# the-lay/voltools

Hardware: AMD Instinct MI355X
Metric: Mvoxels/s, 512^3 f32 filt_bspline StaticVolume transform (resident source, device output) (higher is better)
Workload: dtype f32; 1 GPU; 512^3 float32 filt_bspline, StaticVolume resident in HBM, rotate((0,i,0)) rzxz sweep, output= device buffer; lds_bytes=34816, kernel=8, resident_bytes=1660944384, angles=i

## Files before the change

include/voltools_hip.h:

```cpp
#ifndef VOLTOOLS_HIP_H
#define VOLTOOLS_HIP_H

#include <stddef.h>
#include <stdint.h>

#ifdef __cplusplus
extern "C" {
#endif

enum vt_interp {
    VT_LINEAR = 0,
    VT_BSPLINE = 1,
    VT_BSPLINE_SIMPLE = 2,
    VT_FILT_BSPLINE = 3,
    VT_FILT_BSPLINE_SIMPLE = 4
};

enum vt_flags {
    VT_OUT_DEVICE = 1,
    VT_KEEP_OUTSIDE = 2,
    VT_FORCE_DIRECT = 4,
    VT_FORCE_TILED = 8,
    VT_NO_ZSEP = 16,
    VT_NO_MARCH = 32,
    VT_NO_ZPAIR = 64,
    VT_NO_PACKED = 128,
    VT_FORCE_PACKED = 256,
    VT_FORCE_XSWAP = 512,
    VT_NO_RSWAP = 1024,
    VT_ONESHOT_EDGE_SCIPY = 4096,
    VT_NO_QUAD = 2048,
    VT_NO_BLOCK = 8192,
    VT_NO_ZFIR = 16384,
    VT_NO_REORIENT = 32768,
    VT_NO_ROWS = 65536,
    VT_NO_PLANSHARE = 131072,
    VT_ACCUMULATE = 262144,
    VT_PLACE_DENSE = 524288
};

enum vt_create_flags {
    VT_SRC_DEVICE = 1,
    VT_SLAB_LO_INTERIOR = 2,
    VT_SLAB_HI_INTERIOR = 4,
    VT_EDGE_SCIPY = 16,
    VT_SRC_DEFERRED = 8,
    VT_STACK = 32
};

enum vt_error {
    VT_OK = 0,
    VT_EINVAL = 10001,
    VT_ENODEV = 10002,
    VT_ENOMEM = 10003,
    VT_EUNSUPPORTED = 10004
};

typedef struct vt_volume vt_volume_t;

typedef struct vt_volume_info {
    int32_t device;
    int32_t interp;
    int32_t depth, height, width;
    int32_t out_depth, out_height, out_width;
    int32_t last_kernel;
    int32_t last_tile[3];
    int32_t last_lds_dims[3];
    int32_t last_lds_bytes;
    int32_t last_grid;
    float   prefilter_ms;
    uint64_t resident_bytes;
    float   copies_ms;
    int32_t copies_built;
    int32_t copies_evicted;
    uint64_t max_resident_bytes;
} vt_volume_info_t;

int vt_device_count(int* count);
int vt_device_name(int dev, char* buf, int buflen);
int vt_device_props(int dev, int* cu_count, int* lds_bytes_per_block, uint64_t* hbm_bytes);
int vt_device_synchronize(int dev);

int vt_malloc(int dev, size_t bytes, void** dptr);
int vt_free(int dev, void* dptr);
int vt_memset_zero(int dev, void* dptr, size_t bytes);
int vt_memcpy_h2d(int dev, void* dptr, const void* hptr, size_t bytes);
int vt_memcpy_d2h(int dev, void* hptr, const void* dptr, size_t bytes);
int vt_memcpy_d2d(int dev, void* dst, const void* src, size_t bytes);
int vt_host_register(int dev, void* ptr, size_t bytes);
int vt_host_unregister(int dev, void* ptr);
int vt_device_trim(int dev);

int vt_volume_create(int dev, int depth, int height, int width, int interp,
                     const float* data, int create_flags, vt_volume_t** out);

int vt_volume_create_slab(int dev, int local_depth, int height, int width, int interp,
                          const float* data, int create_flags,
                          int64_t plane0, int64_t global_depth, int64_t out_plane0, int out_depth,
                          vt_volume_t** out);

int vt_volume_upload_planes(vt_volume_t* vol, int first_plane, int nplanes, const float* data, int flags);
int vt_volume_finalize(vt_volume_t* vol);

int vt_has_legacy_kernels(void);

int vt_volume_release_copies(vt_volume_t* vol, uint64_t* freed_bytes);
int vt_volume_set_max_resident(vt_volume_t* vol, uint64_t bytes);
int vt_volume_destroy(vt_volume_t* vol);
int vt_volume_info(const vt_volume_t* vol, vt_volume_info_t* info);
int vt_volume_stream(const vt_volume_t* vol, void** hip_stream);
int vt_volume_sync(vt_volume_t* vol);

int vt_volume_set_output_shape(vt_volume_t* vol, int out_depth, int out_height, int out_width);

int vt_volume_affine(vt_volume_t* vol, const float* m4x4, float* out, int flags);
int vt_volume_affine_f64(vt_volume_t* vol, const double* m4x4, float* out, int flags);

int vt_volume_affine_batch(vt_volume_t* vol, int n, const float* m4x4s, float* out, int flags);

int vt_volume_extract(vt_volume_t* vol, int n, const float* m4x4s,
                      int box_d, int box_h, int box_w, float* out, int flags);
// ... 73 lines not shown
```

voltools_amd/_native.py:

```python
import ctypes
import os
from typing import Optional, Tuple

import numpy as np

_HERE = os.path.dirname(os.path.abspath(__file__))
LIB_PATH = os.environ.get('VT_LIB') or os.path.join(_HERE, 'lib', 'libvoltools_hip.so')

INTERP_CODES = {'linear': 0, 'bspline': 1, 'bspline_simple': 2, 'filt_bspline': 3, 'filt_bspline_simple': 4}

OUT_DEVICE, KEEP_OUTSIDE, FORCE_DIRECT, FORCE_TILED, NO_ZSEP, NO_MARCH, NO_ZPAIR, NO_PACKED, FORCE_PACKED, FORCE_XSWAP, NO_RSWAP, NO_QUAD, ONESHOT_EDGE_SCIPY, NO_BLOCK, NO_ZFIR, NO_REORIENT, NO_ROWS, NO_PLANSHARE, ACCUMULATE, PLACE_DENSE = 1, 2, 4, 8, 16, 32, 64, 128, 256, 512, 1024, 2048, 4096, 8192, 16384, 32768, 65536, 131072, 262144, 524288
SRC_DEVICE, SLAB_LO_INTERIOR, SLAB_HI_INTERIOR, SRC_DEFERRED, EDGE_SCIPY, STACK = 1, 2, 4, 8, 16, 32

SYMBOLS = [
    'vt_device_count', 'vt_device_name', 'vt_device_props', 'vt_device_synchronize',
    'vt_malloc', 'vt_free', 'vt_memset_zero', 'vt_memcpy_h2d', 'vt_memcpy_d2h', 'vt_memcpy_d2d',
    'vt_host_register', 'vt_host_unregister', 'vt_device_trim',
    'vt_volume_create', 'vt_volume_create_slab', 'vt_volume_upload_planes', 'vt_volume_finalize', 'vt_volume_destroy', 'vt_volume_info', 'vt_volume_stream',
    'vt_volume_sync', 'vt_volume_set_output_shape', 'vt_volume_affine', 'vt_volume_affine_f64',
    'vt_volume_project', 'vt_volume_project_f64', 'vt_volume_affine_batch',
    'vt_timer_start', 'vt_timer_stop', 'vt_prefilter_inplace', 'vt_affine_oneshot',
    'vt_last_error', 'vt_version', 'vt_has_legacy_kernels', 'vt_volume_release_copies', 'vt_volume_set_max_resident',
    'vt_volume_extract', 'vt_volume_extract_f64', 'vt_volume_project_batch', 'vt_volume_project_batch_f64',
    'vt_volume_extract_sum', 'vt_volume_extract_sum_f64', 'vt_volume_extract_dot', 'vt_volume_extract_dot_f64',
    'vt_volume_extract_dot_multi', 'vt_volume_extract_dot_multi_f64',
    'vt_volume_extract_sum_multi', 'vt_volume_extract_sum_multi_f64',
    'vt_volume_place', 'vt_volume_place_f64', 'vt_volume_backproject', 'vt_volume_backproject_f64',
    'vt_volume_backproject_boxes', 'vt_volume_backproject_boxes_f64',
    'vt_volume_warp', 'vt_volume_warp_f64',
]


class VolumeInfo(ctypes.Structure):
    _fields_ = [('device', ctypes.c_int32), ('interp', ctypes.c_int32),
                ('depth', ctypes.c_int32), ('height', ctypes.c_int32), ('width', ctypes.c_int32),
                ('out_depth', ctypes.c_int32), ('out_height', ctypes.c_int32), ('out_width', ctypes.c_int32),
                ('last_kernel', ctypes.c_int32), ('last_tile', ctypes.c_int32 * 3),
                ('last_lds_dims', ctypes.c_int32 * 3), ('last_lds_bytes', ctypes.c_int32),
                ('last_grid', ctypes.c_int32), ('prefilter_ms', ctypes.c_float),
                ('resident_bytes', ctypes.c_uint64), ('copies_ms', ctypes.c_float), ('copies_built', ctypes.c_int32),
                ('copies_evicted', ctypes.c_int32), ('max_resident_bytes', ctypes.c_uint64)]


_lib = None


def _preload_hip_runtime():
    import importlib.util
    import sys
    if os.environ.get('VT_HIP_RUNTIME', '') == 'system' or 'torch' in sys.modules:
        return
    try:
        spec = importlib.util.find_spec('torch')
    except (ImportError, ValueError):
        spec = None
    if spec is None or not spec.submodule_search_locations:
        return
    cand = os.path.join(list(spec.submodule_search_locations)[0], 'lib', 'libamdhip64.so')
    if os.path.exists(cand):
        try:
            ctypes.CDLL(cand, mode=ctypes.RTLD_GLOBAL)
        except OSError:
            pass


def load():
    global _lib
    if _lib is not None:
        return _lib
    if not os.path.exists(LIB_PATH):
        raise OSError(f'{LIB_PATH} not found (run __graft_entry__.build())')
    _preload_hip_runtime()
    L = ctypes.CDLL(LIB_PATH)
    c_int, c_void_p, c_size_t, c_i64 = ctypes.c_int, ctypes.c_void_p, ctypes.c_size_t, ctypes.c_int64
    P = ctypes.POINTER
    L.vt_has_legacy_kernels.argtypes = []
    L.vt_device_count.argtypes = [P(c_int)]
    L.vt_device_name.argtypes = [c_int, ctypes.c_char_p, c_int]
    L.vt_device_props.argtypes = [c_int, P(c_int), P(c_int), P(ctypes.c_uint64)]
    L.vt_device_synchronize.argtypes = [c_int]
    L.vt_malloc.argtypes = [c_int, c_size_t, P(c_void_p)]
    L.vt_free.argtypes = [c_int, c_void_p]
    L.vt_memset_zero.argtypes = [c_int, c_void_p, c_size_t]
    L.vt_memcpy_h2d.argtypes = [c_int, c_void_p, c_void_p, c_size_t]
    L.vt_memcpy_d2h.argtypes = [c_int, c_void_p, c_void_p, c_size_t]
    L.vt_host_register.argtypes = [c_int, c_void_p, c_size_t]
    L.vt_host_unregister.argtypes = [c_int, c_void_p]
    L.vt_device_trim.argtypes = [c_int]
    L.vt_memcpy_d2d.argtypes = [c_int, c_void_p, c_void_p, c_size_t]
    L.vt_volume_create.argtypes = [c_int, c_int, c_int, c_int, c_int, c_void_p, c_int, P(c_void_p)]
    L.vt_volume_create_slab.argtypes = [c_int, c_int, c_int, c_int, c_int, c_void_p, c_int,
                                        c_i64, c_i64, c_i64, c_int, P(c_void_p)]
    L.vt_volume_upload_planes.argtypes = [c_void_p, c_int, c_int, c_void_p, c_int]
    L.vt_volume_finalize.argtypes = [c_void_p]
# ... 262 lines not shown
```

voltools_amd/csrc/vt_kernels_block.hip:

```cpp
#include "vt_internal.h"
#include "vt_device.h"

#include <algorithm>
#include <type_traits>

namespace vt {

typedef float v2f __attribute__((ext_vector_type(2)));

constexpr int kBlkTD = 8, kBlkTW = 16;
constexpr int block_max_it(int th) { return th == 16 ? 20 : 13; }

template <int OFF>
__device__ __forceinline__ void lds_read_b64(v2f& r, unsigned a)
{
    asm volatile("ds_read_b64 %0, %1 offset:%2" : "=v"(r) : "v"(a), "n"(OFF));
}

__device__ __forceinline__ v2f pk_fma(v2f a, float w, v2f c) { return __builtin_elementwise_fma(a, (v2f)(w), c); }

__device__ __forceinline__ void bspline_weights_pk(float f, v2f& w30, v2f& w12)
{
    const v2f fg = {f, 1.0f - f};
    const v2f sq = fg * fg;
// ... 14 lines not shown
    } else {
        v2f a30, a12;
        bspline_weights_pk(fx, a30, a12); wx[0] = a30.y; wx[1] = a12.x; wx[2] = a12.y; wx[3] = a30.x;
        bspline_weights_pk(fy, a30, a12); wy[0] = a30.y; wy[1] = a12.x; wy[2] = a12.y; wy[3] = a30.x;
        bspline_weights_pk(fz, a30, a12); wz[0] = a30.y; wz[1] = a12.x; wz[2] = a12.y; wz[3] = a30.x;
    }
    unsigned a[4];
    a[0] = a0; a[1] = a0 + ps4; a[2] = a[1] + ps4; a[3] = a[2] + ps4;

    v2f t[2][6];
#define VT_BLK_ISSUE(c, h, r)                                                                                                   \
    lds_read_b64<(2 * h) * RS4>(r[0], a[c]); lds_read_b64<(2 * h) * RS4 + 8>(r[1], a[c]); lds_read_b64<(2 * h) * RS4 + 16>(r[2], a[c]);     \
    lds_read_b64<(2 * h + 1) * RS4>(r[3], a[c]); lds_read_b64<(2 * h + 1) * RS4 + 8>(r[4], a[c]); lds_read_b64<(2 * h + 1) * RS4 + 16>(r[5], a[c]);
#define VT_BLK_WAIT(n, r) \
    asm volatile("s_waitcnt lgkmcnt(" #n ")" : "+v"(r[0]), "+v"(r[1]), "+v"(r[2]), "+v"(r[3]), "+v"(r[4]), "+v"(r[5]));
#define VT_BLK_SUM(c, h, r)                                                                       \
    {                                                                                             \
        const float w0 = wz[c] * wy[2 * h], w1 = wz[c] * wy[2 * h + 1];                           \
        S0 = pk_fma(r[0], w0, S0); S1 = pk_fma(r[1], w0, S1); S2 = pk_fma(r[2], w0, S2);          \
        S0 = pk_fma(r[3], w1, S0); S1 = pk_fma(r[4], w1, S1); S2 = pk_fma(r[5], w1, S2);          \
    }
    v2f S0 = {0.f, 0.f}, S1 = {0.f, 0.f}, S2 = {0.f, 0.f};
#define VT_BLK_WAITN(r) VT_BLK_WAIT(6, r)
    VT_BLK_ISSUE(0, 0, t[0])
    VT_BLK_ISSUE(0, 1, t[1]) VT_BLK_WAITN(t[0]) VT_BLK_SUM(0, 0, t[0])
    VT_BLK_ISSUE(1, 0, t[0]) VT_BLK_WAITN(t[1]) VT_BLK_SUM(0, 1, t[1])
    VT_BLK_ISSUE(1, 1, t[1]) VT_BLK_WAITN(t[0]) VT_BLK_SUM(1, 0, t[0])
    VT_BLK_ISSUE(2, 0, t[0]) VT_BLK_WAITN(t[1]) VT_BLK_SUM(1, 1, t[1])
    VT_BLK_ISSUE(2, 1, t[1]) VT_BLK_WAITN(t[0]) VT_BLK_SUM(2, 0, t[0])
    VT_BLK_ISSUE(3, 0, t[0]) VT_BLK_WAITN(t[1]) VT_BLK_SUM(2, 1, t[1])
    VT_BLK_ISSUE(3, 1, t[1]) VT_BLK_WAITN(t[0]) VT_BLK_SUM(3, 0, t[0])
    VT_BLK_WAIT(0, t[1]) VT_BLK_SUM(3, 1, t[1])
#undef VT_BLK_WAITN
#undef VT_BLK_ISSUE
#undef VT_BLK_WAIT
#undef VT_BLK_SUM
    const float t0 = par ? S0.y : S0.x, t1 = par ? S1.x : S0.y, t2 = par ? S1.y : S1.x, t3 = par ? S2.x : S1.y;
    return fmaf(wx[3], t3, fmaf(wx[2], t2, fmaf(wx[1], t1, wx[0] * t0)));
}

template <int RS>
__device__ __forceinline__ void stage_block_checked_box(float* lds, const float* __restrict__ src, const float* __restrict__ zeros16,
                                                        const AffineParams& p, const int (&o)[3], int total, int psv, int nvx_used, int tid)
{
    constexpr int nvx = RS / 4;
    const int wave_first = __builtin_amdgcn_readfirstlane(tid & ~63);
    for (int vb = wave_first; vb < total; vb += 256) {
        const int v = vb + (tid & 63);
        const int z = v / psv, rem = v - z * psv;
        const int y = rem / nvx, cx = rem - y * nvx;
        const int gz = o[0] + z, gy = o[1] + y, gx = o[2] + 4 * cx;
        const bool inb = (y < p.Ly) && (cx < nvx_used) && (unsigned)gz < (unsigned)p.sD && (unsigned)gy < (unsigned)p.sH &&
                         (unsigned)gx < (unsigned)p.sP;
        const float* g = inb ? src + (((int64_t)gz * p.sH + gy) * p.sP + gx) : zeros16;
        __builtin_amdgcn_global_load_lds((const __attribute__((address_space(1))) void*)g,
                                         (__attribute__((address_space(3))) void*)(lds + 4 * vb), 16, 0, 0);
    }
}

template <int RS, int MAXIT>
__device__ __forceinline__ void stage_block_checked(float* lds, const float* __restrict__ src, const float* __restrict__ zeros16,
                                                    const AffineParams& p, const int (&o)[3], const int (&voff)[MAXIT], int total, int psv, int tid)
{
    constexpr int nvx = RS / 4;
    const int wave_first = __builtin_amdgcn_readfirstlane(tid & ~63);
    const char* const origin = reinterpret_cast<const char*>(src + (((int64_t)o[0] * p.sH + o[1]) * p.sP + o[2]));
#pragma unroll
    for (int k = 0; k < MAXIT; ++k) {
        if (k * 256 + wave_first < total) {
            int v = k * 256 + tid;
            asm volatile("" : "+v"(v));
            const int z = (int)__umulhi((unsigned)v, p.psv_magic), rem = v - z * psv;
            const int y = rem / nvx, cx = rem - y * nvx;
            const int gz = o[0] + z, gy = o[1] + y, gx = o[2] + 4 * cx;
            const bool inb = (unsigned)gz < (unsigned)p.sD && (unsigned)gy < (unsigned)p.sH && (unsigned)gx < (unsigned)p.sP;
            const float* g = inb ? reinterpret_cast<const float*>(origin + voff[k]) : zeros16;
            if (voff[k] != 0 || v == 0)
                __builtin_amdgcn_global_load_lds((const __attribute__((address_space(1))) void*)g,
                                                 (__attribute__((address_space(3))) void*)(lds + 4 * (k * 256 + wave_first)), 16, 0, 0);
        }
    }
}

template <int KIND, int RS, int TH>
__device__ __forceinline__ void affine_block_body(const float* __restrict__ src, float* __restrict__ out, const float* __restrict__ zeros16,
                                                  int* __restrict__ queue, const AffineParams& p, const PackGeom& geo)
{
    constexpr bool CUBIC = KIND != 0;
    constexpr int HALO = CUBIC ? 1 : 0;
    constexpr int TD = kBlkTD, TW = kBlkTW;
    constexpr int NS = TH == 16 ? 8 : 4;
    constexpr int kBlkMaxIt = block_max_it(TH);
    constexpr bool PIN = TH == 16;
    constexpr int nvx = RS / 4;
    extern __shared__ __attribute__((aligned(16))) float lds[];

    const int tid = threadIdx.x, lane = tid & 63, wv = tid >> 6;
    const int wave_first = __builtin_amdgcn_readfirstlane(tid & ~63);
    const int vd = lane >> 4, vh = 4 * (wv >> 1) + ((lane >> 2) & 3), vw = 4 * (wv & 1) + (lane & 3);
    constexpr int sd[8] = {0, 0, TH == 16 ? 0 : 4, TH == 16 ? 0 : 4, 4, 4, 4, 4};
    constexpr int sh[8] = {0, 0, TH == 16 ? 8 : 0, TH == 16 ? 8 : 0, 8, 8, 0, 0};
    constexpr int sw[8] = {0, 8, 8, 0, 0, 8, 8, 0};
    constexpr int which[7] = {0, TH == 16 ? 1 : 3, 2, 3, 0, 4, 2};

    const int Lz = p.Lz, Ly = p.Ly, ps = p.Lps;
    const int psv = ps >> 2;
    const int total = Lz * psv;
    const int nvx_used = p.Lx_used >> 2;
    const int row_b = p.sP * 4;
    const int plane_b = p.sH * row_b;

    int voff[kBlkMaxIt];
#pragma unroll
    for (int k = 0; k < kBlkMaxIt; ++k) {
        const int v = k * 256 + tid;
        const int z = (int)__umulhi((unsigned)v, p.psv_magic), rem = v - z * psv;
        const int y = rem / nvx, cx = rem - y * nvx;
        bool used = v < total && y < Ly && cx < nvx_used;
        if (used && (p.flags & (1 << 25))) {
            int mn, mx;
            used = packed_row_span(geo, z, y, &mn, &mx);
            used = used && cx >= (mn >> 2) && cx <= (mx >> 2);
        }
        voff[k] = used ? z * plane_b + y * row_b + 16 * cx : 0;
    }

    const bool keep = (p.flags & VT_KEEP_OUTSIDE) != 0;
    const int64_t ostride = (int64_t)p.oH * p.oW;
    const int obase = (int)((vd * ostride + (int64_t)vh * p.oW + vw) * 4);
    const int ostep_d = (int)(4 * ostride * 4), ostep_h = (int)(8 * (int64_t)p.oW * 4);
    const unsigned ps4 = 4u * (unsigned)ps;
    const unsigned lds_base = lds_byte_address(lds);
    int inc_hi[5][3];
    unsigned inc_lo[5][3];
#pragma unroll
    for (int k = 0; k < 5; ++k)
#pragma unroll
        for (int r = 0; r < 3; ++r) {
            inc_hi[k][r] = p.binc_hi[k][r];
            inc_lo[k][r] = p.binc_lo[k][r];
            if (PIN || k == 0 || k == 2 || k == 3) asm volatile("" : "+v"(inc_hi[k][r]), "+v"(inc_lo[k][r]));
        }
    double gm[12], gneg[3], gpos[3], gvlo[3], gvhi[3];
    double mp[3][3];
    const int oc0 = p.ord[0], oc1 = p.ord[1], oc2 = p.ord[2];
    auto load_consts = [&](const auto& kp_) {
        const auto* const kp = &kp_;
#pragma unroll
        for (int i = 0; i < 12; ++i) gm[i] = kp->m[i];
#pragma unroll
        for (int r = 0; r < 3; ++r) { gneg[r] = kp->neg[r]; gpos[r] = kp->pos[r]; gvlo[r] = kp->vlo[r]; gvhi[r] = kp->vhi[r]; }
    };
    auto load_chain = [&](const auto& kp_) {
        const auto* const kp = &kp_;
#pragma unroll
        for (int r = 0; r < 3; ++r) { mp[r][0] = kp->m[4 * r + oc0]; mp[r][1] = kp->m[4 * r + oc1]; mp[r][2] = kp->m[4 * r + oc2]; }
    };
    if constexpr (PIN) {
        load_consts(p);
#pragma unroll
        for (int i = 0; i < 12; ++i) asm volatile("" : "+v"(gm[i]));
#pragma unroll
        for (int r = 0; r < 3; ++r) {
            mp[r][0] = oc0 == 0 ? gm[4 * r] : (oc0 == 1 ? gm[4 * r + 1] : gm[4 * r + 2]);
            mp[r][1] = oc1 == 0 ? gm[4 * r] : (oc1 == 1 ? gm[4 * r + 1] : gm[4 * r + 2]);
            mp[r][2] = oc2 == 0 ? gm[4 * r] : (oc2 == 1 ? gm[4 * r + 1] : gm[4 * r + 2]);
            asm volatile("" : "+v"(gneg[r]), "+v"(gpos[r]), "+v"(gvlo[r]), "+v"(gvhi[r]), "+v"(mp[r][0]), "+v"(mp[r][1]), "+v"(mp[r][2]));
        }
    }
    double toff[3];
#pragma unroll
    for (int r = 0; r < 3; ++r) toff[r] = fma(p.m[4 * r], (double)vd, fma(p.m[4 * r + 1], (double)vh, p.m[4 * r + 2] * (double)vw));
    auto inside_canonical = [&](int d, int h, int w) {
        const double x0 = (double)(oc0 == 0 ? d : (oc0 == 1 ? h : w));
        const double x1 = (double)(oc1 == 0 ? d : (oc1 == 1 ? h : w));
        const double x2 = (double)(oc2 == 0 ? d : (oc2 == 1 ? h : w));
        bool in = true;
#pragma unroll
        for (int r = 0; r < 3; ++r) {
            const double sc = fma(mp[r][0], x0, fma(mp[r][1], x1, fma(mp[r][2], x2, gm[4 * r + 3])));
            in = in && (sc >= gvlo[r]) && (sc < gvhi[r]);
        }
        return in;
    };
#ifdef VT_EXPERIMENTS
    const bool no_stores = (p.flags & (1 << 21)) != 0, no_loads = (p.flags & (1 << 22)) != 0, no_lds = (p.flags & (1 << 26)) != 0;
#else
    constexpr bool no_stores = false, no_loads = false, no_lds = false;
#endif

    int* const ctrl = reinterpret_cast<int*>(lds + (p.lds_cap >> 2));
    const int nids = blocked_tile_count(p.nTd, p.nTh, p.nTw);
    const int nSh = (p.nTh + 3) >> 2, nSw = (p.nTw + 3) >> 2;
    const int xcd = blockIdx.x & 7, per = ((nids >> 6) + 7) / 8 * 64;
    const int id0 = xcd * per, id_cnt = max(0, min(per, nids - id0));
    int* const counter = queue + 32 * xcd;
    const int chunk = p.dch;
    int nxt = 0;
    if (tid == 0) nxt = atomicAdd(counter, chunk);
    int cur = 0, left = 0;
    for (;;) {
        if (left == 0) {
            if (tid == 0) ctrl[0] = nxt;
            __syncthreads();
            cur = ctrl[0];
            left = chunk;
            __syncthreads();
            if (cur >= id_cnt) break;
            if (tid == 0) nxt = atomicAdd(counter, chunk);
        }
        const int id = id0 + cur;
        ++cur; --left;
        if (cur > id_cnt) continue;
        int td_i, th_i, tw_i;
        const unsigned sbi = (unsigned)id >> 6, l6 = (unsigned)id & 63u;
        const unsigned s2 = nSw == 1 ? sbi : __umulhi(sbi, p.nTw_magic), sbw = sbi - s2 * (unsigned)nSw;
        const unsigned sbd = nSh == 1 ? s2 : __umulhi(s2, p.nTh_magic), sbh = s2 - sbd * (unsigned)nSh;
        td_i = (int)(sbd * 4 + (l6 >> 4)); th_i = (int)(sbh * 4 + ((l6 >> 2) & 3)); tw_i = (int)(sbw * 4 + (l6 & 3));
        const bool tile_ok = td_i < p.nTd && th_i < p.nTh && tw_i < p.nTw;
        if (!tile_ok) continue;
        if constexpr (!PIN) {
            typedef const __attribute__((address_space(4))) char* KArg;
            KArg ka = (KArg)__builtin_amdgcn_kernarg_segment_ptr();
            asm volatile("" : "+s"(ka));
            load_consts(*(const __attribute__((address_space(4))) AffineParams*)(ka + 32));
        }
        const int d0 = td_i * TD, h0 = th_i * TH, w0 = tw_i * TW;

        double base[3], lo[3], hi[3];
        bool any_valid = true, all_valid = true;
#pragma unroll
        for (int r = 0; r < 3; ++r) {
            base[r] = fma(gm[4 * r], (double)d0, fma(gm[4 * r + 1], (double)h0, fma(gm[4 * r + 2], (double)w0, gm[4 * r + 3])));
            lo[r] = base[r] + gneg[r];
            hi[r] = base[r] + gpos[r];
            any_valid = any_valid && (hi[r] >= gvlo[r] - kTileMargin) && (lo[r] < gvhi[r] + kTileMargin);
            all_valid = all_valid && (lo[r] >= gvlo[r] + kTileMargin) && (hi[r] < gvhi[r] - kTileMargin);
        }
        float* const otile = out + ((int64_t)d0 * ostride + (int64_t)h0 * p.oW + w0);
        __amdgpu_buffer_rsrc_t orsrc = __builtin_amdgcn_make_buffer_rsrc(reinterpret_cast<char*>(otile), 0, 0x7fffffff, 0x00020000);
        const bool whole = (d0 + TD <= p.oD) && (h0 + TH <= p.oH) && (w0 + TW <= p.oW);

        if (!any_valid) {
            if (!keep) {
#pragma unroll
                for (int s = 0; s < NS; ++s) {
                    const int d = d0 + vd + sd[s], h = h0 + vh + sh[s], w = w0 + vw + sw[s];
                    if (whole || (d < p.oD && h < p.oH && w < p.oW))
                        __builtin_amdgcn_raw_buffer_store_b32(0u, orsrc, obase, (sd[s] >> 2) * ostep_d + (sh[s] >> 3) * ostep_h + 4 * sw[s], 0);
                }
            }
            continue;
        }

        int o[3];
#pragma unroll
        for (int r = 0; r < 3; ++r) o[r] = (int)floor(lo[r]) - HALO;
        o[2] &= ~3;
        const bool box_inside = o[0] >= 0 && o[1] >= 0 && o[2] >= 0 && o[0] + Lz <= p.sD && o[1] + Ly <= p.sH && o[2] + p.Lx_used <= p.sP;

        __syncthreads();
        if (no_loads) {
        } else if (box_inside) {
            __amdgpu_buffer_rsrc_t rsrc = __builtin_amdgcn_make_buffer_rsrc(
                const_cast<char*>(reinterpret_cast<const char*>(src + (((int64_t)o[0] * p.sH + o[1]) * p.sP + o[2]))), 0, 0x7fffffff, 0x00020000);
            char* dst = reinterpret_cast<char*>(lds) + 16 * wave_first;
#pragma unroll
            for (int k = 0; k < kBlkMaxIt; ++k)
                if (k * 256 + wave_first < total)
                    __builtin_amdgcn_raw_ptr_buffer_load_lds(rsrc, (__attribute__((address_space(3))) void*)(dst + 4096 * k), 16, voff[k], 0, 0, 0);
        } else {
            if constexpr (TH == 16) stage_block_checked_box<RS>(lds, src, zeros16, p, o, total, psv, nvx_used, tid);
            else stage_block_checked<RS, kBlkMaxIt>(lds, src, zeros16, p, o, voff, total, psv, tid);
        }
        Fx c[3];
#pragma unroll
        for (int r = 0; r < 3; ++r) c[r] = to_fx((base[r] - (double)o[r]) + toff[r]);
        asm volatile("s_waitcnt vmcnt(0)" ::: "memory");
        __syncthreads();

        unsigned inmask = (1u << NS) - 1u, zmask = 0u;
        if (!(all_valid && whole)) {
            inmask = 0u;
            if constexpr (!PIN) {
                typedef const __attribute__((address_space(4))) char* KArg;
                KArg ka = (KArg)__builtin_amdgcn_kernarg_segment_ptr();
                asm volatile("" : "+s"(ka));
                load_chain(*(const __attribute__((address_space(4))) AffineParams*)(ka + 32));
            }
#pragma unroll
            for (int s = 0; s < NS; ++s) {
                const int d = d0 + vd + sd[s], h = h0 + vh + sh[s], w = w0 + vw + sw[s];
                if (d < p.oD && h < p.oH && w < p.oW) {
                    if (inside_canonical(d, h, w)) inmask |= 1u << s;
                    else if (!keep) zmask |= 1u << s;
                }
            }
        }
#pragma unroll
        for (int s = 0; s < NS; ++s) {
            float val;
            if (no_lds) {
                val = fx_frac(c[0]) + fx_frac(c[1]) + fx_frac(c[2]);
            } else if constexpr (CUBIC) {
                const int x1 = c[2].hi - 1, par = x1 & 1, e = x1 - par;
                const unsigned a0 = lds_base + 4u * (unsigned)(__mul24(c[0].hi - 1, ps) + __mul24(c[1].hi - 1, RS) + e);
                val = cubic_block_sample<KIND == 2, RS>(a0, ps4, par, fx_frac(c[0]), fx_frac(c[1]), fx_frac(c[2]));
            } else {
                const float* q = lds + (__mul24(c[0].hi, ps) + __mul24(c[1].hi, RS) + c[2].hi);
                const float* q1 = q + ps;
                const float fz = fx_frac(c[0]), fy = fx_frac(c[1]), fx = fx_frac(c[2]);
                const float a000 = q[0], a001 = q[1], a010 = q[RS], a011 = q[RS + 1];
                const float a100 = q1[0], a101 = q1[1], a110 = q1[RS], a111 = q1[RS + 1];
                const float x00 = fmaf(fx, a001 - a000, a000);
                const float x01 = fmaf(fx, a011 - a010, a010);
                const float x10 = fmaf(fx, a101 - a100, a100);
                const float x11 = fmaf(fx, a111 - a110, a110);
                const float y0 = fmaf(fy, x01 - x00, x00);
                const float y1 = fmaf(fy, x11 - x10, x10);
                val = fmaf(fz, y1 - y0, y0);
            }
            asm volatile("" : "+v"(val));
            const int soff = (sd[s] >> 2) * ostep_d + (sh[s] >> 3) * ostep_h + 4 * sw[s];
            if (no_stores) {
                if (val == 123.456f) __builtin_amdgcn_raw_buffer_store_b32(__builtin_bit_cast(unsigned, val), orsrc, obase, soff, 0);
            } else if ((inmask >> s) & 1u) {
                __builtin_amdgcn_raw_buffer_store_b32(__builtin_bit_cast(unsigned, val), orsrc, obase, soff, 0);
            } else if ((zmask >> s) & 1u) {
                __builtin_amdgcn_raw_buffer_store_b32(0u, orsrc, obase, soff, 0);
            }
            if (s < NS - 1) {
#pragma unroll
                for (int r = 0; r < 3; ++r) fx_step(c[r], inc_hi[which[s]][r], inc_lo[which[s]][r]);
            }
            asm volatile("" : "+v"(c[0].hi), "+v"(c[0].lo), "+v"(c[1].hi), "+v"(c[1].lo), "+v"(c[2].hi), "+v"(c[2].lo));
        }
    }
    if (tid == 0) {
        __threadfence();
        if (atomicAdd(&queue[256], 1) == (int)gridDim.x - 1) {
#pragma unroll
            for (int i = 0; i < 9; ++i) queue[32 * i] = 0;
        }
    }
}

template <int KIND, int RS>
__global__ __launch_bounds__(256, 2) void affine_block(const float* __restrict__ src, float* __restrict__ out, const float* __restrict__ zeros16,
                                                        int* __restrict__ queue, const AffineParams p, const PackGeom geo)
{
    affine_block_body<KIND, RS, 16>(src, out, zeros16, queue, p, geo);
}
template <int KIND, int RS>
__global__ __launch_bounds__(256, 4) void affine_block_half(const float* __restrict__ src, float* __restrict__ out, const float* __restrict__ zeros16,
                                                             int* __restrict__ queue, const AffineParams p, const PackGeom geo)
{
    affine_block_body<KIND, RS, 8>(src, out, zeros16, queue, p, geo);
}

typedef void (*block_fn)(const float*, float*, const float*, int*, const AffineParams, const PackGeom);

static const int kBlkRS[] = {28, 36, 32, 12, 20, 16, 24};
static const int kOrder16[] = {0, 1, 2};
static const int kOrder8[] = {3, 4, 0, 1, 5, 6, 2};
int block_rs_count() { return (int)(sizeof(kBlkRS) / sizeof(kBlkRS[0])); }
int block_rs(int idx) { return kBlkRS[idx]; }
int block_rs_order(int th, const int** order) { *order = th == 16 ? kOrder16 : kOrder8; return th == 16 ? 3 : 7; }
int block_max_vectors(int th) { return 256 * block_max_it(th); }
void block_tile(int th, int* td, int* tw) { (void)th; *td = kBlkTD; *tw = kBlkTW; }

template <int RS, int TH>
static block_fn pick_block_kind(int kind)
{
    if constexpr (TH == 16) {
        switch (kind) {
            case 0: return affine_block<0, RS>;
            case 1: return affine_block<1, RS>;
            default: return affine_block<2, RS>;
        }
    } else {
        switch (kind) {
            case 0: return affine_block_half<0, RS>;
            case 1: return affine_block_half<1, RS>;
            default: return affine_block_half<2, RS>;
        }
    }
}

static block_fn block_entry(int rs_idx, int kind, int th)
{
    if (th == 16) return rs_idx == 0 ? pick_block_kind<28, 16>(kind) : (rs_idx == 1 ? pick_block_kind<36, 16>(kind) : pick_block_kind<32, 16>(kind));
    switch (rs_idx) {
        case 0: return pick_block_kind<28, 8>(kind);
        case 1: return pick_block_kind<36, 8>(kind);
        case 2: return pick_block_kind<32, 8>(kind);
        case 3: return pick_block_kind<12, 8>(kind);
        case 4: return pick_block_kind<20, 8>(kind);
        case 5: return pick_block_kind<16, 8>(kind);
        default: return pick_block_kind<24, 8>(kind);
    }
}

hipError_t init_block_kernels()
{
    for (int th = 8; th <= 16; th += 8)
        for (int rs = 0; rs < (th == 16 ? 3 : block_rs_count()); ++rs)
            for (int kind = 0; kind < 3; ++kind) {
                hipError_t e = hipFuncSetAttribute(reinterpret_cast<const void*>(block_entry(rs, kind, th)),
                                                   hipFuncAttributeMaxDynamicSharedMemorySize, 160 * 1024);
                if (e != hipSuccess) return e;
            }
    return hipSuccess;
}

hipError_t launch_affine_block(int rs_idx, int th, int interp, const float* src, float* out, const float* zeros16, int* queue,
                               const AffineParams& p, const PackGeom& geo, int grid, int lds_bytes, hipStream_t stream)
{
    hipLaunchKernelGGL(block_entry(rs_idx, interp_kind(interp), th), dim3(grid), dim3(256), lds_bytes, stream, src, out, zeros16, queue, p, geo);
    return hipGetLastError();
}

}
```

voltools_amd/csrc/vt_plan.hip:

```cpp
#include "vt_host.h"
#include "vt_device.h"

#include <cmath>
#include <cstring>

namespace vt {
namespace {

struct PlanCtx {
    const vt_volume* v;
    const double* m;
    int flags;
    AffineParams* p;
    TilePlan* plan;
    bool cubic;
    bool zsep;
    int halo2;
};

#ifdef VT_LEGACY
int64_t round_aware_chunks(int64_t oD, int g, int64_t inplane, int64_t resident, int64_t n0, int extra, int min_dch, int64_t n_floor)
{
    if (resident <= 0 || inplane > resident || inplane * n0 >= 16 * resident) return n0;
    auto cost = [&](int64_t n) {
// ... 686 lines not shown
            int f[3];
            for (int r = 0; r < 3; ++r)
                f[r] = (int)std::floor(kBase[b][r] + 24.0 + m[4 * r] * t[0] + m[4 * r + 1] * t[1] + m[4 * r + 2] * t[2]);
            const int a = f[0] * PS + f[1] * RS + (cubic ? (((f[2] - 1) & ~1) >> 1) * 2 : f[2]);
            const int word = cubic ? (a >> 1) : a;
            bool seen = false;
            for (int i = 0; i < n; ++i) seen = seen || words[i] == word;
            if (!seen) words[n++] = word;
        }
        int cnt[32] = {0}, worst = 0;
        for (int i = 0; i < n; ++i) worst = std::max(worst, ++cnt[((words[i] % 32) + 32) % 32]);
        tot += worst;
    }
    return tot / 4.0;
}

bool plan_block_th(PlanCtx& c, int th);

bool plan_block(PlanCtx& c)
{
    if (c.v->tune.block_th == 8 && plan_block_th(c, 8)) return true;
    return plan_block_th(c, 16);
}

bool plan_block_th(PlanCtx& c, int th)
{
    const vt_volume* v = c.v;
    const double* m = c.m;
    AffineParams* p = c.p;
    TilePlan* plan = c.plan;
    if ((c.flags & (VT_NO_BLOCK | VT_NO_PACKED | VT_FORCE_PACKED)) || v->tune.no_block) return false;
    if (c.zsep) return false;
    if (!c.cubic && !v->tune.block_linear) return false;
    if (!(c.flags & VT_FORCE_TILED) && (int64_t)v->oD * v->oH * v->oW < (int64_t)v->tune.block_min * v->tune.block_min * v->tune.block_min) return false;
    int T[3];
    T[1] = th;
    block_tile(th, &T[0], &T[2]);
    int L[3];
    for (int r = 0; r < 3; ++r) {
        double ext = 0;
        for (int k = 0; k < 3; ++k) ext += std::fabs(m[4 * r + k]) * (T[k] - 1);
        if (!(ext < 256.0)) return false;
        L[r] = (int)std::floor(ext) + 3 + c.halo2;
    }
    const int lx_used = (L[2] + 3 + 3) & ~3;
    int rs_idx = -1, RS = 0, PS = 0;
    int64_t vectors = 0;
    auto try_rs = [&](int idx) {
        if (idx < 0 || idx >= block_rs_count() || (th == 16 && idx > 2) || block_rs(idx) < lx_used) return false;
        const int rs = block_rs(idx);
        int best_pad = 0;
        double best_f = 1e300;
        for (int pad = 0; pad < 64; pad += 4) {
            if ((int64_t)L[0] * (L[1] * rs + pad) / 4 > block_max_vectors(th)) break;
            const double f = block_conflicts(m, 0, rs, L[1] * rs + pad, c.cubic) * (1.0 + 0.002 * pad);
            if (f < best_f - 1e-9) { best_f = f; best_pad = pad; }
        }
        if (v->tune.block_pad >= 0) best_pad = v->tune.block_pad & ~3;
        const int ps = L[1] * rs + best_pad;
        const int64_t vec = (int64_t)L[0] * ps / 4;
        if (vec > block_max_vectors(th)) return false;
        rs_idx = idx; RS = rs; PS = ps; vectors = vec;
        return true;
    };
    if (v->tune.block_rs >= 0) {
        if (!try_rs(v->tune.block_rs)) return false;
    } else {
        const int* order = nullptr;
        const int norder = block_rs_order(th, &order);
        bool ok = false;
        for (int i = 0; i < norder && !ok; ++i) ok = try_rs(order[i]);
        if (!ok) return false;
    }
    const int64_t plane_b = (int64_t)v->H * v->P * 4;
    if ((int64_t)L[0] * plane_b >= 0x7fffffffLL || (int64_t)T[0] * v->oH * v->oW * 4 >= 0x7fffffffLL) return false;
    const int box_bytes = (int)((vectors + 63) / 64 * 64 * 16);
    const int lds_bytes = box_bytes + 16;
    if (lds_bytes > v->lds_limit) return false;

    plan->kind = 9; plan->cfg = rs_idx; plan->td = T[0]; plan->th = T[1]; plan->tw = T[2];
    plan->lds_bytes = lds_bytes;
    p->Lz = L[0]; p->Ly = L[1]; p->Lx = RS; p->Lx_used = lx_used; p->Lps = PS;
    p->flags = (c.flags & VT_KEEP_OUTSIDE) | experiment_flags(v);
    set_tile_reach(p, m, T, 0);
    double inv[9];
    if (!v->tune.block_no_trim && invert3(m, inv)) {
        PackGeom& g = plan->geo;
        for (int i = 0; i < 9; ++i) g.inv[i] = inv[i];
        for (int cc = 0; cc < 3; ++cc) g.cst[cc] = inv[3 * cc] * p->neg[0] + inv[3 * cc + 1] * p->neg[1] + inv[3 * cc + 2] * p->neg[2];
        for (int r = 0; r < 3; ++r) {
            g.ext[r] = p->pos[r] - p->neg[r];
            g.T[r] = T[r];
        }
        g.halo = c.cubic ? 1 : 0;
        g.Lxbox = lx_used;
        g.Lybox = L[1];
        p->flags |= (1 << 25);
    }
    p->nTd = (v->oD + T[0] - 1) / T[0];
    p->nTh = (v->oH + T[1] - 1) / T[1];
    p->nTw = (v->oW + T[2] - 1) / T[2];
    p->psv_magic = (uint32_t)(4294967296.0 / (double)(PS / 4)) + 1u;
    p->lds_cap = box_bytes;
    p->nTw_magic = (uint32_t)((1ULL << 32) / (uint64_t)((p->nTw + 3) >> 2) + 1);
    p->nTh_magic = (uint32_t)((1ULL << 32) / (uint64_t)((p->nTh + 3) >> 2) + 1);
    const int col[5] = {2, 1, 2, 0, 1};
    const double mul[5] = {8.0, 8.0, -8.0, 4.0, -8.0};
    const int neg_of[5] = {-1, -1, 0, -1, 1};
    for (int s = 0; s < 5; ++s)
        for (int r = 0; r < 3; ++r) {
            if (neg_of[s] >= 0) {
                const uint64_t fwd = ((uint64_t)(uint32_t)p->binc_hi[neg_of[s]][r] << 32) | p->binc_lo[neg_of[s]][r];
                const uint64_t back = 0 - fwd;
                p->binc_hi[s][r] = (int32_t)(uint32_t)(back >> 32); p->binc_lo[s][r] = (uint32_t)back;
                continue;
            }
            const double step = m[4 * r + col[s]] * mul[s];
            const double fl = std::floor(step);
            double lo = std::floor((step - fl) * 4294967296.0 + 0.5);
            int32_t hi = (int32_t)fl;
            if (lo >= 4294967296.0) { lo = 0; hi += 1; }
            p->binc_hi[s][r] = hi; p->binc_lo[s][r] = (uint32_t)lo;
        }
    plan->blocks_per_cu = (int)std::min<int64_t>(th == 16 ? 2 : 4, (160 * 1024) / lds_bytes);
    const int64_t ids = blocked_tile_count(p->nTd, p->nTh, p->nTw);
    int64_t grid = std::min<int64_t>((int64_t)v->cu_count * plan->blocks_per_cu, ids);
    grid = std::max<int64_t>(8, (grid + 7) / 8 * 8);
    p->dch = (int)std::max<int64_t>(1, std::min<int64_t>(4, ids / (grid * 8)));
    plan->grid = (int)grid;
    return true;
}

bool plan_general(PlanCtx& c)
{
    double box_bpv = 1e300;
    const bool have_box = pick_box_tile(c, &box_bpv);
    if (plan_packed(c, have_box, box_bpv)) return true;
    if (!have_box) return false;
    const double* mm = c.m;
    const double det = mm[0] * (mm[5] * mm[10] - mm[6] * mm[9]) - mm[1] * (mm[4] * mm[10] - mm[6] * mm[8]) + mm[2] * (mm[4] * mm[9] - mm[5] * mm[8]);
    if (c.plan->kind == 2 && !(c.flags & VT_FORCE_TILED) && c.v->tune.tile < 0 && std::fabs(det) >= 9.0 &&
        (c.plan->lds_bytes > 80 * 1024 || (!c.cubic && box_bpv > 43.0))) {
        c.plan->kind = 1; c.plan->cfg = -1; c.plan->td = c.plan->th = c.plan->tw = 0; c.plan->lds_bytes = 0; c.plan->grid = 0;
        return true;
    }
    if (!finish_box(c)) { c.plan->kind = 1; }
    return true;
}

typedef bool (*plan_fn)(PlanCtx&);
struct Family { const char* name; plan_fn plan; };
const Family kFamilies[] = {
    {"quad", plan_quad},
#ifdef VT_LEGACY
    {"zpair", plan_zpair},
    {"march", plan_march},
#endif
    {"block", plan_block},
    {"general", plan_general},
};

}

static void plan_prepare(const vt_volume* v, const double m[12], int flags, AffineParams* p, TilePlan* plan)
{
    std::memcpy(p->m, m, sizeof(double) * 12);
// ... 123 lines not shown
```

Baseline: 711,300 Mvoxels/s.

## Defer block tile output stores to overlap them with the next tile's LDS staging

For the TH=8 block kernel, each tile's computed values are now held in registers and written out only after the next tile's buffer loads to LDS have been issued. A counted vmcnt wait lets the outstanding stores stay in flight during the barrier, so store latency overlaps the next load. It also skips load instructions for waves with no used vectors and makes the box base address wave-uniform with readfirstlane. This costs extra registers, which may hurt occupancy, and adds an opt-out flag plus a doubled set of kernel instantiations.

```diff
diff --git a/include/voltools_hip.h b/include/voltools_hip.h
--- a/include/voltools_hip.h
+++ b/include/voltools_hip.h
@@ -36,7 +36,8 @@
     VT_NO_ROWS = 65536,
     VT_NO_PLANSHARE = 131072,
     VT_ACCUMULATE = 262144,
-    VT_PLACE_DENSE = 524288
+    VT_PLACE_DENSE = 524288,
+    VT_NO_BLOCKPIPE = 1048576
 };
 
 enum vt_create_flags {
diff --git a/voltools_amd/_native.py b/voltools_amd/_native.py
--- a/voltools_amd/_native.py
+++ b/voltools_amd/_native.py
@@ -9,7 +9,7 @@
 
 INTERP_CODES = {'linear': 0, 'bspline': 1, 'bspline_simple': 2, 'filt_bspline': 3, 'filt_bspline_simple': 4}
 
-OUT_DEVICE, KEEP_OUTSIDE, FORCE_DIRECT, FORCE_TILED, NO_ZSEP, NO_MARCH, NO_ZPAIR, NO_PACKED, FORCE_PACKED, FORCE_XSWAP, NO_RSWAP, NO_QUAD, ONESHOT_EDGE_SCIPY, NO_BLOCK, NO_ZFIR, NO_REORIENT, NO_ROWS, NO_PLANSHARE, ACCUMULATE, PLACE_DENSE = 1, 2, 4, 8, 16, 32, 64, 128, 256, 512, 1024, 2048, 4096, 8192, 16384, 32768, 65536, 131072, 262144, 524288
+OUT_DEVICE, KEEP_OUTSIDE, FORCE_DIRECT, FORCE_TILED, NO_ZSEP, NO_MARCH, NO_ZPAIR, NO_PACKED, FORCE_PACKED, FORCE_XSWAP, NO_RSWAP, NO_QUAD, ONESHOT_EDGE_SCIPY, NO_BLOCK, NO_ZFIR, NO_REORIENT, NO_ROWS, NO_PLANSHARE, ACCUMULATE, PLACE_DENSE, NO_BLOCKPIPE = 1, 2, 4, 8, 16, 32, 64, 128, 256, 512, 1024, 2048, 4096, 8192, 16384, 32768, 65536, 131072, 262144, 524288, 1048576
 SRC_DEVICE, SLAB_LO_INTERIOR, SLAB_HI_INTERIOR, SRC_DEFERRED, EDGE_SCIPY, STACK = 1, 2, 4, 8, 16, 32
 
 SYMBOLS = [
diff --git a/voltools_amd/csrc/vt_kernels_block.hip b/voltools_amd/csrc/vt_kernels_block.hip
--- a/voltools_amd/csrc/vt_kernels_block.hip
+++ b/voltools_amd/csrc/vt_kernels_block.hip
@@ -120,7 +120,7 @@
     }
 }
 
-template <int KIND, int RS, int TH>
+template <int KIND, int RS, int TH, bool PIPED>
 __device__ __forceinline__ void affine_block_body(const float* __restrict__ src, float* __restrict__ out, const float* __restrict__ zeros16,
                                                   int* __restrict__ queue, const AffineParams& p, const PackGeom& geo)
 {
@@ -162,6 +162,13 @@
         }
         voff[k] = used ? z * plane_b + y * row_b + 16 * cx : 0;
     }
+    constexpr bool PIPE = TH == 8 && PIPED;
+    unsigned wave_used = 0u;
+    if constexpr (PIPE) {
+#pragma unroll
+        for (int k = 0; k < kBlkMaxIt; ++k)
+            if (__builtin_amdgcn_ballot_w64(voff[k] != 0 || (k == 0 && tid == 0)) != 0) wave_used |= 1u << k;
+    }
 
     const bool keep = (p.flags & VT_KEEP_OUTSIDE) != 0;
     const int64_t ostride = (int64_t)p.oH * p.oW;
@@ -177,7 +184,7 @@
         for (int r = 0; r < 3; ++r) {
             inc_hi[k][r] = p.binc_hi[k][r];
             inc_lo[k][r] = p.binc_lo[k][r];
-            if (PIN || k == 0 || k == 2 || k == 3) asm volatile("" : "+v"(inc_hi[k][r]), "+v"(inc_lo[k][r]));
+            if (PIN || k == 0 || k == 2 || (k == 3 && !PIPE)) asm volatile("" : "+v"(inc_hi[k][r]), "+v"(inc_lo[k][r]));
         }
     double gm[12], gneg[3], gpos[3], gvlo[3], gvhi[3];
     double mp[3][3];
@@ -226,6 +233,7 @@
 #else
     constexpr bool no_stores = false, no_loads = false, no_lds = false;
 #endif
+    const bool legacy = !PIPE || no_stores;
 
     int* const ctrl = reinterpret_cast<int*>(lds + (p.lds_cap >> 2));
     const int nids = blocked_tile_count(p.nTd, p.nTh, p.nTw);
@@ -237,6 +245,38 @@
     int nxt = 0;
     if (tid == 0) nxt = atomicAdd(counter, chunk);
     int cur = 0, left = 0;
+    float pval[NS];
+    unsigned pmask = 0u;
+    float* ptile = out;
+    int pend = 0;
+#pragma unroll
+    for (int s = 0; s < NS; ++s) pval[s] = 0.f;
+    auto issue_pending = [&]() -> int {
+        int n = 0;
+        if (pend != 0) {
+            __amdgpu_buffer_rsrc_t prsrc = __builtin_amdgcn_make_buffer_rsrc(reinterpret_cast<char*>(ptile), 0, 0x7fffffff, 0x00020000);
+            if (pend == 1) {
+#pragma unroll
+                for (int s = 0; s < NS; ++s)
+                    __builtin_amdgcn_raw_buffer_store_b32(__builtin_bit_cast(unsigned, pval[s]), prsrc, obase,
+                                                          (sd[s] >> 2) * ostep_d + (sh[s] >> 3) * ostep_h + 4 * sw[s], 0);
+                n = NS;
+            } else {
+#pragma unroll
+                for (int s = 0; s < NS; ++s) {
+                    const bool in = (pmask >> s) & 1u, st = ((pmask | (pmask >> 8)) >> s) & 1u;
+                    if (__builtin_amdgcn_ballot_w64(st) != 0) {
+                        if (st)
+                            __builtin_amdgcn_raw_buffer_store_b32(in ? __builtin_bit_cast(unsigned, pval[s]) : 0u, prsrc, obase,
+                                                                  (sd[s] >> 2) * ostep_d + (sh[s] >> 3) * ostep_h + 4 * sw[s], 0);
+                        ++n;
+                    }
+                }
+            }
+            pend = 0;
+        }
+        return n;
+    };
     for (;;) {
         if (left == 0) {
             if (tid == 0) ctrl[0] = nxt;
@@ -280,6 +320,7 @@
         const bool whole = (d0 + TD <= p.oD) && (h0 + TH <= p.oH) && (w0 + TW <= p.oW);
 
         if (!any_valid) {
+            if constexpr (PIPE) issue_pending();
             if (!keep) {
 #pragma unroll
                 for (int s = 0; s < NS; ++s) {
@@ -300,13 +341,27 @@
         __syncthreads();
         if (no_loads) {
         } else if (box_inside) {
-            __amdgpu_buffer_rsrc_t rsrc = __builtin_amdgcn_make_buffer_rsrc(
-                const_cast<char*>(reinterpret_cast<const char*>(src + (((int64_t)o[0] * p.sH + o[1]) * p.sP + o[2]))), 0, 0x7fffffff, 0x00020000);
+            const char* box0 = reinterpret_cast<const char*>(src + (((int64_t)o[0] * p.sH + o[1]) * p.sP + o[2]));
+            if constexpr (PIPE) {
+                const uint64_t a = reinterpret_cast<uint64_t>(box0);
+                box0 = reinterpret_cast<const char*>(((uint64_t)(unsigned)__builtin_amdgcn_readfirstlane((int)(a >> 32)) << 32) |
+                                                     (unsigned)__builtin_amdgcn_readfirstlane((int)(unsigned)a));
+            }
+            __amdgpu_buffer_rsrc_t rsrc = __builtin_amdgcn_make_buffer_rsrc(const_cast<char*>(box0), 0, 0x7fffffff, 0x00020000);
             char* dst = reinterpret_cast<char*>(lds) + 16 * wave_first;
-#pragma unroll
-            for (int k = 0; k < kBlkMaxIt; ++k)
-                if (k * 256 + wave_first < total)
-                    __builtin_amdgcn_raw_ptr_buffer_load_lds(rsrc, (__attribute__((address_space(3))) void*)(dst + 4096 * k), 16, voff[k], 0, 0, 0);
+            if (legacy) {
+#pragma unroll
+                for (int k = 0; k < kBlkMaxIt; ++k)
+                    if (k * 256 + wave_first < total)
+                        __builtin_amdgcn_raw_ptr_buffer_load_lds(rsrc, (__attribute__((address_space(3))) void*)(dst + 4096 * k), 16, voff[k], 0, 0, 0);
+            } else {
+#pragma unroll
+                for (int k = 0; k < kBlkMaxIt; ++k)
+                    if ((wave_used >> k) & 1u) {
+                        if (voff[k] != 0 || (k == 0 && tid == 0))
+                            __builtin_amdgcn_raw_ptr_buffer_load_lds(rsrc, (__attribute__((address_space(3))) void*)(dst + 4096 * k), 16, voff[k], 0, 0, 0);
+                    }
+            }
         } else {
             if constexpr (TH == 16) stage_block_checked_box<RS>(lds, src, zeros16, p, o, total, psv, nvx_used, tid);
             else stage_block_checked<RS, kBlkMaxIt>(lds, src, zeros16, p, o, voff, total, psv, tid);
@@ -314,8 +369,23 @@
         Fx c[3];
 #pragma unroll
         for (int r = 0; r < 3; ++r) c[r] = to_fx((base[r] - (double)o[r]) + toff[r]);
-        asm volatile("s_waitcnt vmcnt(0)" ::: "memory");
-        __syncthreads();
+        if (legacy) {
+            asm volatile("s_waitcnt vmcnt(0)" ::: "memory");
+            __syncthreads();
+        } else {
+            asm volatile("" ::: "memory");
+            const int nst = __builtin_amdgcn_readfirstlane(issue_pending());
+            static_assert(NS <= 4 || !PIPE, "the counted wait covers four store instructions");
+            switch (nst) {
+                case 0: asm volatile("s_waitcnt vmcnt(0)" ::: "memory"); break;
+                case 1: asm volatile("s_waitcnt vmcnt(1)" ::: "memory"); break;
+                case 2: asm volatile("s_waitcnt vmcnt(2)" ::: "memory"); break;
+                case 3: asm volatile("s_waitcnt vmcnt(3)" ::: "memory"); break;
+                default: asm volatile("s_waitcnt vmcnt(4)" ::: "memory"); break;
+            }
+            __builtin_amdgcn_s_barrier();
+            asm volatile("" ::: "memory");
+        }
 
         unsigned inmask = (1u << NS) - 1u, zmask = 0u;
         if (!(all_valid && whole)) {
@@ -360,7 +430,9 @@
             }
             asm volatile("" : "+v"(val));
             const int soff = (sd[s] >> 2) * ostep_d + (sh[s] >> 3) * ostep_h + 4 * sw[s];
-            if (no_stores) {
+            if (!legacy) {
+                pval[s] = val;
+            } else if (no_stores) {
                 if (val == 123.456f) __builtin_amdgcn_raw_buffer_store_b32(__builtin_bit_cast(unsigned, val), orsrc, obase, soff, 0);
             } else if ((inmask >> s) & 1u) {
                 __builtin_amdgcn_raw_buffer_store_b32(__builtin_bit_cast(unsigned, val), orsrc, obase, soff, 0);
@@ -373,7 +445,13 @@
             }
             asm volatile("" : "+v"(c[0].hi), "+v"(c[0].lo), "+v"(c[1].hi), "+v"(c[1].lo), "+v"(c[2].hi), "+v"(c[2].lo));
         }
-    }
+        if (!legacy) {
+            pmask = inmask | (zmask << 8);
+            ptile = otile;
+            pend = (all_valid && whole) ? 1 : 2;
+        }
+    }
+    if constexpr (PIPE) issue_pending();
     if (tid == 0) {
         __threadfence();
         if (atomicAdd(&queue[256], 1) == (int)gridDim.x - 1) {
@@ -387,13 +465,13 @@
 __global__ __launch_bounds__(256, 2) void affine_block(const float* __restrict__ src, float* __restrict__ out, const float* __restrict__ zeros16,
                                                         int* __restrict__ queue, const AffineParams p, const PackGeom geo)
 {
-    affine_block_body<KIND, RS, 16>(src, out, zeros16, queue, p, geo);
-}
-template <int KIND, int RS>
+    affine_block_body<KIND, RS, 16, false>(src, out, zeros16, queue, p, geo);
+}
+template <int KIND, int RS, bool PIPED>
 __global__ __launch_bounds__(256, 4) void affine_block_half(const float* __restrict__ src, float* __restrict__ out, const float* __restrict__ zeros16,
                                                              int* __restrict__ queue, const AffineParams p, const PackGeom geo)
 {
-    affine_block_body<KIND, RS, 8>(src, out, zeros16, queue, p, geo);
+    affine_block_body<KIND, RS, 8, PIPED>(src, out, zeros16, queue, p, geo);
 }
 
 typedef void (*block_fn)(const float*, float*, const float*, int*, const AffineParams, const PackGeom);
@@ -407,7 +485,7 @@
 int block_max_vectors(int th) { return 256 * block_max_it(th); }
 void block_tile(int th, int* td, int* tw) { (void)th; *td = kBlkTD; *tw = kBlkTW; }
 
-template <int RS, int TH>
+template <int RS, int TH, bool PIPED>
 static block_fn pick_block_kind(int kind)
 {
     if constexpr (TH == 16) {
@@ -418,43 +496,51 @@
         }
     } else {
         switch (kind) {
-            case 0: return affine_block_half<0, RS>;
-            case 1: return affine_block_half<1, RS>;
-            default: return affine_block_half<2, RS>;
-        }
-    }
-}
-
-static block_fn block_entry(int rs_idx, int kind, int th)
-{
-    if (th == 16) return rs_idx == 0 ? pick_block_kind<28, 16>(kind) : (rs_idx == 1 ? pick_block_kind<36, 16>(kind) : pick_block_kind<32, 16>(kind));
+            case 0: return affine_block_half<0, RS, PIPED>;
+            case 1: return affine_block_half<1, RS, PIPED>;
+            default: return affine_block_half<2, RS, PIPED>;
+        }
+    }
+}
+
+template <bool PIPED>
+static block_fn block_entry_half(int rs_idx, int kind)
+{
     switch (rs_idx) {
-        case 0: return pick_block_kind<28, 8>(kind);
-        case 1: return pick_block_kind<36, 8>(kind);
-        case 2: return pick_block_kind<32, 8>(kind);
-        case 3: return pick_block_kind<12, 8>(kind);
-        case 4: return pick_block_kind<20, 8>(kind);
-        case 5: return pick_block_kind<16, 8>(kind);
-        default: return pick_block_kind<24, 8>(kind);
-    }
+        case 0: return pick_block_kind<28, 8, PIPED>(kind);
+        case 1: return pick_block_kind<36, 8, PIPED>(kind);
+        case 2: return pick_block_kind<32, 8, PIPED>(kind);
+        case 3: return pick_block_kind<12, 8, PIPED>(kind);
+        case 4: return pick_block_kind<20, 8, PIPED>(kind);
+        case 5: return pick_block_kind<16, 8, PIPED>(kind);
+        default: return pick_block_kind<24, 8, PIPED>(kind);
+    }
+}
+
+static block_fn block_entry(int rs_idx, int kind, int th, bool piped)
+{
+    if (th == 16)
+        return rs_idx == 0 ? pick_block_kind<28, 16, false>(kind) : (rs_idx == 1 ? pick_block_kind<36, 16, false>(kind) : pick_block_kind<32, 16, false>(kind));
+    return piped ? block_entry_half<true>(rs_idx, kind) : block_entry_half<false>(rs_idx, kind);
 }
 
 hipError_t init_block_kernels()
 {
     for (int th = 8; th <= 16; th += 8)
         for (int rs = 0; rs < (th == 16 ? 3 : block_rs_count()); ++rs)
-            for (int kind = 0; kind < 3; ++kind) {
-                hipError_t e = hipFuncSetAttribute(reinterpret_cast<const void*>(block_entry(rs, kind, th)),
-                                                   hipFuncAttributeMaxDynamicSharedMemorySize, 160 * 1024);
-                if (e != hipSuccess) return e;
-            }
+            for (int kind = 0; kind < 3; ++kind)
+                for (int piped = 0; piped < (th == 16 ? 1 : 2); ++piped) {
+                    hipError_t e = hipFuncSetAttribute(reinterpret_cast<const void*>(block_entry(rs, kind, th, piped != 0)),
+                                                       hipFuncAttributeMaxDynamicSharedMemorySize, 160 * 1024);
+                    if (e != hipSuccess) return e;
+                }
     return hipSuccess;
 }
 
 hipError_t launch_affine_block(int rs_idx, int th, int interp, const float* src, float* out, const float* zeros16, int* queue,
                                const AffineParams& p, const PackGeom& geo, int grid, int lds_bytes, hipStream_t stream)
 {
-    hipLaunchKernelGGL(block_entry(rs_idx, interp_kind(interp), th), dim3(grid), dim3(256), lds_bytes, stream, src, out, zeros16, queue, p, geo);
+    hipLaunchKernelGGL(block_entry(rs_idx, interp_kind(interp), th, !(p.flags & (1 << 24))), dim3(grid), dim3(256), lds_bytes, stream, src, out, zeros16, queue, p, geo);
     return hipGetLastError();
 }
 
diff --git a/voltools_amd/csrc/vt_plan.hip b/voltools_amd/csrc/vt_plan.hip
--- a/voltools_amd/csrc/vt_plan.hip
+++ b/voltools_amd/csrc/vt_plan.hip
@@ -792,6 +792,7 @@
     plan->lds_bytes = lds_bytes;
     p->Lz = L[0]; p->Ly = L[1]; p->Lx = RS; p->Lx_used = lx_used; p->Lps = PS;
     p->flags = (c.flags & VT_KEEP_OUTSIDE) | experiment_flags(v);
+    if (c.flags & VT_NO_BLOCKPIPE) p->flags |= (1 << 24);
     set_tile_reach(p, m, T, 0);
     double inv[9];
     if (!v->tune.block_no_trim && invert3(m, inv)) {
```

Measured after the change: 711,300 Mvoxels/s, median of 2. No clear change (+0.0%).
